# minhtrangvy/distributed_bitcoin_minter

Measured on AMD Instinct MI355X. Metric: GH/s (SHA-256 "msg nonce" min-search) at 1/2/4/8 MI355X; % of int32 VALU peak, higher is better.
Workload: dtype u32

## Files before the change

### distributed_bitcoin_minter_amd/csrc/bm_kernels.hpp

```cpp
#pragma once
#include <hip/hip_runtime.h>

#include <cstdint>
#include <type_traits>

#include "bm_common.h"
#include "bm_sha256.hpp"

namespace bm {

#define BM_DEV __device__ __forceinline__

template <int B, int E, class F>
BM_DEV void static_for(F&& f) {
    if constexpr (B < E) {
        f(std::integral_constant<int, B>{});
        static_for<B + 1, E>(f);
    }
}

BM_DEV uint32_t rotr(uint32_t x, uint32_t n) { return __builtin_amdgcn_alignbit(x, x, n); }

BM_DEV uint32_t xor3(uint32_t a, uint32_t b, uint32_t c) {
    if (__builtin_constant_p(a) && __builtin_constant_p(b) && __builtin_constant_p(c)) return a ^ b ^ c;
    return __builtin_amdgcn_bitop3_b32(a, b, c, 0x96);
}
BM_DEV uint32_t ch(uint32_t e, uint32_t f, uint32_t g) {
    if (__builtin_constant_p(e) && __builtin_constant_p(f) && __builtin_constant_p(g)) return (e & f) ^ (~e & g);
    return __builtin_amdgcn_bitop3_b32(e, f, g, 0xCA);
}
BM_DEV uint32_t maj(uint32_t a, uint32_t b, uint32_t c) {
    if (__builtin_constant_p(a) && __builtin_constant_p(b) && __builtin_constant_p(c))
        return (a & b) ^ (a & c) ^ (b & c);
    return __builtin_amdgcn_bitop3_b32(a, b, c, 0xE8);
}
BM_DEV uint32_t bsig0(uint32_t a) { return xor3(rotr(a, 2), rotr(a, 13), rotr(a, 22)); }
BM_DEV uint32_t bsig1(uint32_t e) { return xor3(rotr(e, 6), rotr(e, 11), rotr(e, 25)); }
BM_DEV uint32_t ssig0(uint32_t x) { return xor3(rotr(x, 7), rotr(x, 18), x >> 3); }
BM_DEV uint32_t ssig1(uint32_t x) { return xor3(rotr(x, 17), rotr(x, 19), x >> 10); }

template <int T>
BM_DEV void sha_round(uint32_t (&s)[8], uint32_t w) {
    uint32_t& a = s[(0 - T) & 7];
    uint32_t& b = s[(1 - T) & 7];
    uint32_t& c = s[(2 - T) & 7];
    uint32_t& d = s[(3 - T) & 7];
    uint32_t& e = s[(4 - T) & 7];
    uint32_t& f = s[(5 - T) & 7];
    uint32_t& g = s[(6 - T) & 7];
    uint32_t& h = s[(7 - T) & 7];
    const uint32_t t1 = h + bsig1(e) + ch(e, f, g) + (kK256[T] + w);
    d += t1;
    h = t1 + bsig0(a) + maj(a, b, c);
}

#ifndef BM_PAD_ADD3S
#define BM_PAD_ADD3S 1
#endif

BM_DEV uint32_t add3_sgpr(uint32_t a, uint32_t s, uint32_t b) {
    uint32_t r;
    asm("v_add3_u32 %0, %1, %2, %3" : "=v"(r) : "v"(a), "s"(s), "v"(b));
    return r;
}

template <int T, bool KW_SGPR = false>
BM_DEV void sha_round_kw(uint32_t (&s)[8], uint32_t kw) {
    uint32_t& a = s[(0 - T) & 7];
    uint32_t& b = s[(1 - T) & 7];
    uint32_t& c = s[(2 - T) & 7];
    uint32_t& d = s[(3 - T) & 7];
    uint32_t& e = s[(4 - T) & 7];
    uint32_t& f = s[(5 - T) & 7];
    uint32_t& g = s[(6 - T) & 7];
    uint32_t& h = s[(7 - T) & 7];
    uint32_t t1;
    if constexpr (KW_SGPR && BM_PAD_ADD3S)
        t1 = add3_sgpr(h, kw, ch(e, f, g)) + bsig1(e);
    else
        t1 = h + bsig1(e) + ch(e, f, g) + kw;
    d += t1;
    h = t1 + bsig0(a) + maj(a, b, c);
}

template <int R0, int R1>
BM_DEV void sha_rounds(uint32_t (&s)[8], uint32_t (&w)[16]) {
    static_for<R0, R1>([&](auto I) {
        constexpr int t = decltype(I)::value;
        if constexpr (t >= 16)
            w[t & 15] = ssig1(w[(t - 2) & 15]) + w[(t - 7) & 15] + ssig0(w[(t - 15) & 15]) + w[t & 15];
        sha_round<t>(s, w[t & 15]);
    });
}

BM_DEV uint32_t ssig0_uniform(uint32_t x) {
    return ((x >> 7) | (x << 25)) ^ ((x >> 18) | (x << 14)) ^ (x >> 3);
}

#ifndef BM_PIN
#define BM_PIN 1
#endif

BM_DEV uint32_t ssig0_salu(uint32_t x) {
    uint32_t r, t0, t1, t2;
    asm("s_lshr_b32 %1, %4, 7\n\t"
        "s_lshl_b32 %2, %4, 25\n\t"
        "s_or_b32 %1, %1, %2\n\t"
        "s_lshr_b32 %2, %4, 18\n\t"
        "s_lshl_b32 %3, %4, 14\n\t"
        "s_or_b32 %2, %2, %3\n\t"
        "s_xor_b32 %1, %1, %2\n\t"
        "s_lshr_b32 %2, %4, 3\n\t"
        "s_xor_b32 %0, %1, %2"
        : "=s"(r), "=&s"(t0), "=&s"(t1), "=&s"(t2)
        : "s"(x)
        : "scc");
    return r;
}

BM_DEV uint32_t vgpr_copy(uint32_t x) {
    uint32_t r;
    asm("v_mov_b32 %0, %1" : "=v"(r) : "s"(x));
    return r;
}

template <int R0, int V>
BM_DEV uint32_t sha_rounds_h0(uint32_t (&s)[8], uint32_t (&w)[16], uint32_t s0v, uint32_t h0_add) {
    static_assert(R0 <= V && V >= 1 && V <= 15, "varying word");
    static_for<R0, 63>([&](auto I) {
        constexpr int t = decltype(I)::value;
        if constexpr (t >= 16) {
            uint32_t s0;
            if constexpr (t - 15 == V)
                s0 = s0v;
            else
                s0 = ssig0(w[(t - 15) & 15]);
            w[t & 15] = ssig1(w[(t - 2) & 15]) + w[(t - 7) & 15] + s0 + w[t & 15];
        }
        sha_round<t>(s, w[t & 15]);
    });
    w[15] = ssig1(w[13]) + w[8] + ssig0(w[0]) + w[15];
    const uint32_t a = s[1], b = s[2], c = s[3], e = s[5], f = s[6], g = s[7], h = s[0];
    const uint32_t t1 = h + bsig1(e) + ch(e, f, g) + (kK256[63] + h0_add) + w[15];
    return t1 + bsig0(a) + maj(a, b, c);
}

BM_DEV void sha_compress(uint32_t (&st)[8], uint32_t (&w)[16]) {
    uint32_t s[8];
#pragma unroll
    for (int i = 0; i < 8; ++i) s[i] = st[i];
    sha_rounds<0, 64>(s, w);
#pragma unroll
    for (int i = 0; i < 8; ++i) st[i] += s[i];
}

template <int P, bool PADB>
constexpr int64_t tail_word(int k) {
    constexpr int LW = P / 4;
    if (k == LW + 1 && (P % 4) == 3 && P != 63) return 0x80000000ll;
    if (!PADB && k == 15) return -1;
    return 0;
}

template <int P, int NBV>
BM_DEV void add_task_digits(uint32_t (&W)[16 * NBV], uint64_t t, uint32_t ms, uint32_t nd) {
    uint64_t x = t;
    static_for<1, 20>([&](auto I) {
        constexpr int i = decltype(I)::value;
        constexpr int pos = 64 * (NBV - 1) + P - i;
        if constexpr (pos >= 0) {
            if (i >= (int)ms && i < (int)nd) {
                const uint64_t q = x / 10u;
                const uint32_t d = (uint32_t)(x - q * 10u);
                x = q;
                W[pos >> 2] += d << (8 * (3 - (pos & 3)));
            }
        }
    });
}

BM_DEV bool lex_less(uint64_t h1, uint64_t n1, uint64_t h2, uint64_t n2) {
    return h1 < h2 || (h1 == h2 && n1 < n2);
}

template <int XOR>
BM_DEV uint64_t swizzle_xor_u64(uint64_t v) {
    constexpr int pat = (XOR << 10) | 0x1F;
    const uint32_t lo = (uint32_t)__builtin_amdgcn_ds_swizzle((int)(uint32_t)v, pat);
    const uint32_t hi = (uint32_t)__builtin_amdgcn_ds_swizzle((int)(uint32_t)(v >> 32), pat);
    return ((uint64_t)hi << 32) | lo;
}

BM_DEV uint64_t readlane_u64(uint64_t v, int lane) {
    const uint32_t lo = (uint32_t)__builtin_amdgcn_readlane((int)(uint32_t)v, lane);
    const uint32_t hi = (uint32_t)__builtin_amdgcn_readlane((int)(uint32_t)(v >> 32), lane);
    return ((uint64_t)hi << 32) | lo;
}

BM_DEV void wave_min(uint64_t& h, uint64_t& n) {
    static_for<0, 5>([&](auto I) {
        constexpr int x = 1 << decltype(I)::value;
        const uint64_t oh = swizzle_xor_u64<x>(h), on = swizzle_xor_u64<x>(n);
        if (lex_less(oh, on, h, n)) {
            h = oh;
            n = on;
        }
    });
    const uint64_t h0 = readlane_u64(h, 0), n0 = readlane_u64(n, 0);
    const uint64_t h1 = readlane_u64(h, 32), n1 = readlane_u64(n, 32);
    if (lex_less(h1, n1, h0, n0)) {
        h = h1;
        n = n1;
    } else {
        h = h0;
        n = n0;
    }
}

template <int NT>
BM_DEV bool block_min(uint64_t& h, uint64_t& n) {
    constexpr int NWAVE = NT / 64;
    __shared__ Partial sh[NWAVE];
    wave_min(h, n);
    const int wave = threadIdx.x >> 6;
    if ((threadIdx.x & 63) == 0) sh[wave] = Partial{h, n};
    __syncthreads();
    if (threadIdx.x == 0) {
#pragma unroll
        for (int i = 1; i < NWAVE; ++i)
            if (lex_less(sh[i].hash, sh[i].nonce, h, n)) {
                h = sh[i].hash;
                n = sh[i].nonce;
            }
        return true;
    }
    return false;
}

BM_DEV uint64_t readfirstlane_u64(uint64_t v) {
    const uint32_t lo = (uint32_t)__builtin_amdgcn_readfirstlane((int)(uint32_t)v);
    const uint32_t hi = (uint32_t)__builtin_amdgcn_readfirstlane((int)(uint32_t)(v >> 32));
    return ((uint64_t)hi << 32) | lo;
}

#ifndef BM_FOLD
#define BM_FOLD 1
#endif
#ifndef BM_WAVES_MAIN
#define BM_WAVES_MAIN 7
#endif
#ifndef BM_WAVES_PAD
#define BM_WAVES_PAD 5
#endif
#ifndef BM_WAVES_NBV2
#define BM_WAVES_NBV2 7
#endif
#ifndef BM_NBV2_TIGHT
#define BM_NBV2_TIGHT 1
#endif
constexpr bool nbv2_tight(int P) { return BM_NBV2_TIGHT && P == 4; }
constexpr int search_waves(int P, int NBV) {
    return (NBV == 1 && P >= 55) ? BM_WAVES_PAD
                                 : (NBV == 2 ? (nbv2_tight(P) ? 6 : BM_WAVES_NBV2) : BM_WAVES_MAIN);
}
#ifndef BM_LDS_BEST
#define BM_LDS_BEST 0
#endif
#ifndef BM_CLOCK_PROBE
#define BM_CLOCK_PROBE 0
#endif
constexpr int kClockSlot = 16;
#ifndef BM_KATTR
#define BM_KATTR __attribute__((amdgpu_waves_per_eu(search_waves(P, NBV), 8)))
#endif

template <int P, int NBV, int PADK, bool TGT = false, bool HITS = false>
BM_DEV void search_body(const SearchArgs& A, Partial* __restrict__ part, unsigned long long* __restrict__ counter,
                        uint64_t target = 0, unsigned long long* hit = nullptr, Partial* hit_buf = nullptr,
                        uint64_t hit_cap = 0) {
    static_assert(!(TGT || HITS) || PADK == -1, "target and hits modes run the generic kernels");
    static_assert(!(TGT && HITS), "one mode");
    static_assert(P >= 0 && P < 64 && (NBV == 1 || (NBV == 2 && P <= 18)), "layout");
    constexpr int LW = P / 4;
    constexpr int BOFF = 16 * (NBV - 1);
    constexpr bool PADB = (NBV == 1) && (P >= 55);
    constexpr bool PADC = PADK >= 0;
    static_assert(!PADC || (PADB && PADK <= kMaxPadPrefixBlocks), "PADK is a padding-block layout");
    constexpr bool TWOW = (P % 4 == 0) && (LW >= 1);
    constexpr bool kFold = BM_FOLD && !PADB && LW >= 1 && !(NBV == 1 && (P == 53 || P == 54)) &&
                           !(NBV == 2 && P >= 17);
    constexpr bool kPin = BM_PIN && kFold && !(NBV == 1 && P >= 48);

    constexpr uint32_t inc0 = 1u << (8 * (3 - P % 4));
    constexpr uint32_t inc1 = (P % 4) >= 1 ? 1u << (8 * (4 - P % 4)) : 0u;
    constexpr uint32_t inc2 = (P % 4) >= 2 ? 1u << (8 * (5 - P % 4)) : 0u;
    constexpr uint32_t inc3 = (P % 4) >= 3 ? 1u << (8 * (6 - P % 4)) : 0u;

    uint64_t best_h = ~0ull, best_n = ~0ull;
    uint32_t bh = 0xFFFFFFFFu;
    const uint32_t thi = (uint32_t)(target >> 32);
    (void)thi;
#if BM_LDS_BEST
    __shared__ uint64_t lbest_h[kBlock], lbest_n[kBlock];
    lbest_h[threadIdx.x] = ~0ull;
    lbest_n[threadIdx.x] = ~0ull;
#endif

    const uint32_t S = A.S;
    const uint32_t n_in = TWOW ? 10u : S;
    const uint32_t n_out = TWOW ? S / 10u : 1u;
    const uint32_t lane = threadIdx.x & 63;
    const uint64_t ntask = A.t_end - A.t0;
    const uint64_t chunk = 64ull * A.chunk_m;

    if (BM_CLOCK_PROBE && blockIdx.x == 0 && threadIdx.x == 0) {
        counter[kClockSlot + 0] = __builtin_amdgcn_s_memtime();
        counter[kClockSlot + 1] = __builtin_amdgcn_s_memrealtime();
    }
    for (;;) {
        uint64_t base = 0;
        if constexpr (TGT) {
            uint64_t seen = 0;
            if (lane == 0) {
                base = atomicAdd(counter, (unsigned long long)chunk);
                seen = __hip_atomic_load(hit, __ATOMIC_RELAXED, __HIP_MEMORY_SCOPE_AGENT);
            }
            base = readfirstlane_u64(base);
            if (base >= ntask) break;
            seen = readfirstlane_u64(seen);
            if (seen < A.nonce_base || seen - A.nonce_base < (A.t0 + base) * (uint64_t)S) break;
        } else {
            if (lane == 0) base = atomicAdd(counter, (unsigned long long)chunk);
            base = readfirstlane_u64(base);
            if (base >= ntask) break;
        }
        for (uint32_t i = 0; i < A.chunk_m; ++i) {
            const uint64_t tt = base + 64ull * i + lane;
            if (tt >= ntask) break;
            const uint64_t t = A.t0 + tt;

            uint32_t W[16 * NBV];
            static_for<0, 16 * NBV>([&](auto K) { W[decltype(K)::value] = A.tmpl[decltype(K)::value]; });
            add_task_digits<P, NBV>(W, t, A.ms, A.nd);

            uint32_t st[8];
#pragma unroll
            for (int q = 0; q < 8; ++q) st[q] = PADK == 0 ? kIV256[q] : A.mid[q];
            if constexpr (NBV == 2) {
                uint32_t wa[16];
#pragma unroll
                for (int k = 0; k < 16; ++k) wa[k] = W[k];
                sha_compress(st, wa);
            }

            uint32_t wb[16];
            static_for<0, 16>([&](auto K) {
                constexpr int k = decltype(K)::value;
                if constexpr (k <= LW) {
                    wb[k] = W[BOFF + k];
                } else {
                    constexpr int64_t c = tail_word<P, PADB>(k);
                    if constexpr (c < 0)
                        wb[k] = (kPin && NBV == 1) ? vgpr_copy(A.tmpl[BOFF + k]) : A.tmpl[BOFF + k];
                    else
                        wb[k] = (uint32_t)c;
                }
            });
            constexpr int R0 = TWOW ? LW - 1 : LW;
            uint32_t s00[8];
#pragma unroll
            for (int q = 0; q < 8; ++q) s00[q] = st[q];
            sha_rounds<0, R0>(s00, wb);

            const uint64_t vbase = t * (uint64_t)S;
            for (uint32_t jo = 0; jo < n_out; ++jo) {
                uint32_t wo[16];
#pragma unroll
                for (int k = 0; k < 16; ++k) wo[k] = wb[k];
                uint32_t s0[8];
#pragma unroll
                for (int q = 0; q < 8; ++q) s0[q] = s00[q];
                if constexpr (TWOW) {
                    wo[LW - 1] = wb[LW - 1] + jo;
                    sha_rounds<LW - 1, LW>(s0, wo);
                }
                const uint32_t wl = wo[LW];
                const uint32_t s0wl = ssig0(wl);
                const uint32_t h0_add = (kPin && NBV == 1) ? vgpr_copy(st[0]) : st[0];
                const uint32_t h1_add = (kPin && NBV == 1) ? vgpr_copy(st[1]) : st[1];

                uint32_t J = 0, c0 = 0, c1 = 0, c2 = 0;
                for (uint32_t j = 0; j < n_in; ++j) {
                    uint32_t w[16];
#pragma unroll
                    for (int k = 0; k < 16; ++k) w[k] = wo[k];
                    w[LW] = wl + J;
                    uint32_t x[8];
#pragma unroll
                    for (int q = 0; q < 8; ++q) x[q] = s0[q];

                    uint32_t h0, h1;
                    if constexpr (kFold) {
                        const uint32_t s0J = kPin ? ssig0_salu(J) : ssig0_uniform(J);
                        h0 = sha_rounds_h0<LW, LW>(x, w, s0wl ^ s0J, h0_add);
                        h1 = h1_add + x[1];
                    } else if constexpr (PADB) {
                        sha_rounds<LW, 64>(x, w);
                        uint32_t y[8];
#pragma unroll
                        for (int q = 0; q < 8; ++q) y[q] = st[q] + x[q];
                        uint32_t z[8];
#pragma unroll
                        for (int q = 0; q < 8; ++q) z[q] = y[q];
                        static_for<0, 64>([&](auto I) {
                            constexpr int tt2 = decltype(I)::value;
                            if constexpr (PADC) {
                                constexpr uint32_t kw = kPadKW<P, (PADK > 0 ? PADK : 0)>.v[tt2];
                                sha_round_kw<tt2>(z, kw);
                            } else {
                                sha_round_kw<tt2, true>(z, A.padkw[tt2]);
                            }
                        });
                        h0 = y[0] + z[0];
                        h1 = y[1] + z[1];
                    } else {
                        sha_rounds<LW, 64>(x, w);
                        h0 = st[0] + x[0];
                        h1 = st[1] + x[1];
                    }

                    if (__builtin_expect(h0 <= bh, 0)) {
                        const uint64_t h = ((uint64_t)h0 << 32) | h1;
                        const uint64_t v = vbase + (uint64_t)jo * n_in + j;
                        if constexpr (TGT) {
                            if (h <= target && v >= A.vlo && v <= A.vhi)
                                atomicMin(hit, (unsigned long long)(A.nonce_base + v));
                        }
                        if constexpr (HITS) {
                            if (h <= target && v >= A.vlo && v <= A.vhi) {
                                const unsigned long long idx = atomicAdd(hit, 1ull);
                                if (idx < hit_cap) {
                                    using u64x2 = unsigned long long __attribute__((ext_vector_type(2)));
                                    *reinterpret_cast<u64x2*>(hit_buf + idx) = u64x2{h, A.nonce_base + v};
                                }
                            }
                        }
#if BM_LDS_BEST
                        if (h < lbest_h[threadIdx.x] && v >= A.vlo && v <= A.vhi) {
                            lbest_h[threadIdx.x] = h;
                            lbest_n[threadIdx.x] = A.nonce_base + v;
                            bh = HITS ? (h0 > thi ? h0 : thi) : h0;
                        }
#else
                        if (h < best_h && v >= A.vlo && v <= A.vhi) {
                            best_h = h;
                            best_n = A.nonce_base + v;
                            bh = HITS ? (h0 > thi ? h0 : thi) : h0;
                        }
#endif
                    }

                    J += inc0;
                    if (++c0 == 10u) {
                        c0 = 0;
                        J += inc1 - 10u * inc0;
                        if (++c1 == 10u) {
                            c1 = 0;
                            J += inc2 - 10u * inc1;
                            if (++c2 == 10u) {
                                c2 = 0;
                                J += inc3 - 10u * inc2;
                            }
                        }
                    }
                }
            }
        }
    }

    if (BM_CLOCK_PROBE && blockIdx.x == 0 && threadIdx.x == 0) {
        counter[kClockSlot + 2] = __builtin_amdgcn_s_memtime();
        counter[kClockSlot + 3] = __builtin_amdgcn_s_memrealtime();
    }
#if BM_LDS_BEST
    best_h = lbest_h[threadIdx.x];
    best_n = lbest_n[threadIdx.x];
#endif
    if (block_min<kBlock>(best_h, best_n)) part[A.part_off + blockIdx.x] = Partial{best_h, best_n};
}

template <int P, int NBV>
__global__ __launch_bounds__(kBlock) BM_KATTR void search_kernel(
    const SearchArgs A, Partial* __restrict__ part, unsigned long long* __restrict__ counter) {
    search_body<P, NBV, -1>(A, part, counter);
}

template <int P, int NBV = 1>
__global__ __launch_bounds__(kBlock) BM_KATTR void search_kernel_padc(
    const SearchArgs A, Partial* __restrict__ part, unsigned long long* __restrict__ counter) {
    static_assert(NBV == 1 && P >= 55, "padding-block layouts only");
    search_body<P, 1, 0>(A, part, counter);
}

template <int P, int K, int NBV = 1>
__global__ __launch_bounds__(kBlock) BM_KATTR void search_kernel_padk(
    const SearchArgs A, Partial* __restrict__ part, unsigned long long* __restrict__ counter) {
    static_assert(NBV == 1 && P >= 55 && K >= 1 && K <= kMaxPadPrefixBlocks, "padding-block layouts only");
    search_body<P, 1, K>(A, part, counter);
}

template <int P, int NBV>
__global__ __launch_bounds__(kBlock) BM_KATTR void target_kernel(
    const SearchArgs A, Partial* __restrict__ part, unsigned long long* __restrict__ counter, const uint64_t target,
    unsigned long long* __restrict__ hit) {
    search_body<P, NBV, -1, true>(A, part, counter, target, hit);
}

template <int P, int NBV>
__global__ __launch_bounds__(kBlock) BM_KATTR void hits_kernel(
    const SearchArgs A, Partial* __restrict__ part, unsigned long long* __restrict__ counter, const uint64_t target,
    unsigned long long* __restrict__ hit_count, Partial* __restrict__ hit_buf, const uint64_t hit_cap) {
    search_body<P, NBV, -1, false, true>(A, part, counter, target, hit_count, hit_buf, hit_cap);
}

}
```

Before: 52.28.

## Compute task digits once per wave and share best-hash threshold across lanes

```diff
diff --git a/distributed_bitcoin_minter_amd/csrc/bm_digits.hpp b/distributed_bitcoin_minter_amd/csrc/bm_digits.hpp
--- /dev/null
+++ b/distributed_bitcoin_minter_amd/csrc/bm_digits.hpp
@@ -0,0 +1,115 @@
+#pragma once
+#include <cstdint>
+
+#if defined(__HIPCC__) || defined(__CUDACC__)
+#define BM_DIGITS_FN __host__ __device__ __forceinline__
+#else
+#define BM_DIGITS_FN inline
+#endif
+#if defined(__clang__)
+#define BM_UNROLL _Pragma("unroll")
+#else
+#define BM_UNROLL
+#endif
+
+namespace bm {
+
+constexpr int kDigitWords = 5;
+
+constexpr int task_digit_words(int P, int NBV) {
+    const int E = 64 * (NBV - 1) + P;
+    return ((E < 19 ? E : 19) + 3) / 4;
+}
+
+BM_DIGITS_FN void pack9(uint32_t x, uint64_t& lo8, uint32_t& d8) {
+    uint64_t p = 0;
+    BM_UNROLL
+    for (int k = 0; k < 8; ++k) {
+        const uint32_t q = x / 10u;
+        p |= (uint64_t)(x - q * 10u) << (8 * k);
+        x = q;
+    }
+    lo8 = p;
+    d8 = x;
+}
+
+template <int NW>
+BM_DIGITS_FN void task_digits_uniform(uint64_t u, uint32_t (&T)[kDigitWords]) {
+    BM_UNROLL
+    for (int k = 0; k < kDigitWords; ++k) T[k] = 0;
+    if (NW == 0) return;
+    uint32_t l0, l1 = 0, l2 = 0;
+    if (NW < 3 || u < 1000000000ull) {
+        l0 = (uint32_t)u;
+    } else {
+        const uint64_t q = u / 1000000000ull;
+        l0 = (uint32_t)(u - q * 1000000000ull);
+        if (q < 1000000000ull) {
+            l1 = (uint32_t)q;
+        } else {
+            l2 = (uint32_t)(q / 1000000000ull);
+            l1 = (uint32_t)(q - (uint64_t)l2 * 1000000000ull);
+        }
+    }
+    uint64_t p0;
+    uint32_t e0;
+    pack9(l0, p0, e0);
+    T[0] = (uint32_t)p0;
+    T[1] = (uint32_t)(p0 >> 32);
+    T[2] = e0;
+    if (NW >= 3 && (l1 | l2) != 0) {
+        uint64_t p1;
+        uint32_t e1;
+        pack9(l1, p1, e1);
+        const uint32_t q2 = l2 / 10u;
+        T[2] |= (uint32_t)p1 << 8;
+        T[3] = (uint32_t)(p1 >> 24);
+        T[4] = (uint32_t)(p1 >> 56) | (e1 << 8) | ((l2 - q2 * 10u) << 16) | (q2 << 24);
+    }
+}
+
+BM_DIGITS_FN uint32_t lane_digits(uint32_t lane) {
+    const uint32_t q = lane / 10u;
+    return (lane - q * 10u) | (q << 8);
+}
+
+template <int NW>
+BM_DIGITS_FN void task_digits_add_lane(const uint32_t (&T)[kDigitWords], uint32_t lane2, uint32_t (&R)[kDigitWords]) {
+    uint32_t carry = 0;
+    BM_UNROLL
+    for (int k = 0; k < kDigitWords; ++k) {
+        if (k >= NW) {
+            R[k] = 0;
+            continue;
+        }
+        const uint64_t s = (uint64_t)T[k] + (k == 0 ? lane2 : 0u) + 0xF6F6F6F6u + carry;
+        carry = (uint32_t)(s >> 32);
+        const uint32_t x = (uint32_t)s;
+        const uint32_t h = x & 0x80808080u;
+        R[k] = x - (((h - (h >> 7)) | h) & 0xF6F6F6F6u);
+    }
+}
+
+template <int P, int NBV>
+BM_DIGITS_FN void place_task_digits(uint32_t (&W)[16 * NBV], const uint32_t (&R)[kDigitWords], uint32_t ms) {
+    constexpr int E = 64 * (NBV - 1) + P;
+    constexpr int NW = task_digit_words(P, NBV);
+    constexpr int c = 8 * (3 - E % 4);
+    if (NW == 0) return;
+    uint32_t Q[kDigitWords + 1];
+    const uint32_t sh = 32u - 8u * ms;
+    BM_UNROLL
+    for (int k = 0; k <= NW; ++k) {
+        const uint32_t hi = k < NW ? R[k] : 0u, lo = k > 0 ? R[k - 1] : 0u;
+        Q[k] = (uint32_t)((((uint64_t)hi << 32) | lo) >> sh);
+    }
+    BM_UNROLL
+    for (int k = 0; k <= NW + 1; ++k) {
+        const int idx = E / 4 - k;
+        if (idx < 0 || (c == 0 && k > NW)) break;
+        const uint32_t hi = k <= NW ? Q[k] : 0u, lo = k > 0 ? Q[k - 1] : 0u;
+        W[idx] += c == 0 ? hi : (hi << c) | (lo >> ((32 - c) & 31));
+    }
+}
+
+}
diff --git a/distributed_bitcoin_minter_amd/csrc/bm_kernels.hpp b/distributed_bitcoin_minter_amd/csrc/bm_kernels.hpp
--- a/distributed_bitcoin_minter_amd/csrc/bm_kernels.hpp
+++ b/distributed_bitcoin_minter_amd/csrc/bm_kernels.hpp
@@ -5,6 +5,7 @@
 #include <type_traits>
 
 #include "bm_common.h"
+#include "bm_digits.hpp"
 #include "bm_sha256.hpp"
 
 namespace bm {
@@ -163,7 +164,16 @@
 }
 
 template <int P, int NBV>
-BM_DEV void add_task_digits(uint32_t (&W)[16 * NBV], uint64_t t, uint32_t ms, uint32_t nd) {
+BM_DEV void add_task_digits(uint32_t (&W)[16 * NBV], uint64_t u, uint32_t lane2, uint32_t ms) {
+    constexpr int NW = task_digit_words(P, NBV);
+    uint32_t T[kDigitWords], R[kDigitWords];
+    task_digits_uniform<NW>(u, T);
+    task_digits_add_lane<NW>(T, lane2, R);
+    place_task_digits<P, NBV>(W, R, ms);
+}
+
+template <int P, int NBV>
+BM_DEV void add_task_digits_div(uint32_t (&W)[16 * NBV], uint64_t t, uint32_t ms, uint32_t nd) {
     uint64_t x = t;
     static_for<1, 20>([&](auto I) {
         constexpr int i = decltype(I)::value;
@@ -263,6 +273,12 @@
     return (NBV == 1 && P >= 55) ? BM_WAVES_PAD
                                  : (NBV == 2 ? (nbv2_tight(P) ? 6 : BM_WAVES_NBV2) : BM_WAVES_MAIN);
 }
+#ifndef BM_TASK_DIGITS_SALU
+#define BM_TASK_DIGITS_SALU 1
+#endif
+#ifndef BM_WAVE_BH
+#define BM_WAVE_BH 1
+#endif
 #ifndef BM_LDS_BEST
 #define BM_LDS_BEST 0
 #endif
@@ -290,6 +306,8 @@
     constexpr bool kFold = BM_FOLD && !PADB && LW >= 1 && !(NBV == 1 && (P == 53 || P == 54)) &&
                            !(NBV == 2 && P >= 17);
     constexpr bool kPin = BM_PIN && kFold && !(NBV == 1 && P >= 48);
+    constexpr bool kSaluDigits = BM_TASK_DIGITS_SALU && !PADB;
+    constexpr bool kWaveBh = BM_WAVE_BH && !PADB;
 
     constexpr uint32_t inc0 = 1u << (8 * (3 - P % 4));
     constexpr uint32_t inc1 = (P % 4) >= 1 ? 1u << (8 * (4 - P % 4)) : 0u;
@@ -310,6 +328,7 @@
     const uint32_t n_in = TWOW ? 10u : S;
     const uint32_t n_out = TWOW ? S / 10u : 1u;
     const uint32_t lane = threadIdx.x & 63;
+    const uint32_t lane2 = lane_digits(lane);
     const uint64_t ntask = A.t_end - A.t0;
     const uint64_t chunk = 64ull * A.chunk_m;
 
@@ -341,7 +360,10 @@
 
             uint32_t W[16 * NBV];
             static_for<0, 16 * NBV>([&](auto K) { W[decltype(K)::value] = A.tmpl[decltype(K)::value]; });
-            add_task_digits<P, NBV>(W, t, A.ms, A.nd);
+            if constexpr (kSaluDigits)
+                add_task_digits<P, NBV>(W, A.t0 + base + 64ull * i, lane2, A.ms);
+            else
+                add_task_digits_div<P, NBV>(W, t, A.ms, A.nd);
 
             uint32_t st[8];
 #pragma unroll
@@ -429,35 +451,77 @@
                         h1 = st[1] + x[1];
                     }
 
-                    if (__builtin_expect(h0 <= bh, 0)) {
-                        const uint64_t h = ((uint64_t)h0 << 32) | h1;
-                        const uint64_t v = vbase + (uint64_t)jo * n_in + j;
-                        if constexpr (TGT) {
-                            if (h <= target && v >= A.vlo && v <= A.vhi)
-                                atomicMin(hit, (unsigned long long)(A.nonce_base + v));
+                    if constexpr (!kWaveBh) {
+                        if (__builtin_expect(h0 <= bh, 0)) {
+                            const uint64_t h = ((uint64_t)h0 << 32) | h1;
+                            const uint64_t v = vbase + (uint64_t)jo * n_in + j;
+                            if constexpr (TGT) {
+                                if (h <= target && v >= A.vlo && v <= A.vhi)
+                                    atomicMin(hit, (unsigned long long)(A.nonce_base + v));
+                            }
+                            if constexpr (HITS) {
+                                if (h <= target && v >= A.vlo && v <= A.vhi) {
+                                    const unsigned long long idx = atomicAdd(hit, 1ull);
+                                    if (idx < hit_cap) {
+                                        using u64x2 = unsigned long long __attribute__((ext_vector_type(2)));
+                                        *reinterpret_cast<u64x2*>(hit_buf + idx) = u64x2{h, A.nonce_base + v};
+                                    }
+                                }
+                            }
+#if BM_LDS_BEST
+                            if (h < lbest_h[threadIdx.x] && v >= A.vlo && v <= A.vhi) {
+                                lbest_h[threadIdx.x] = h;
+                                lbest_n[threadIdx.x] = A.nonce_base + v;
+                                bh = HITS ? (h0 > thi ? h0 : thi) : h0;
+                            }
+#else
+                            if (h < best_h && v >= A.vlo && v <= A.vhi) {
+                                best_h = h;
+                                best_n = A.nonce_base + v;
+                                bh = HITS ? (h0 > thi ? h0 : thi) : h0;
+                            }
+#endif
                         }
-                        if constexpr (HITS) {
-                            if (h <= target && v >= A.vlo && v <= A.vhi) {
-                                const unsigned long long idx = atomicAdd(hit, 1ull);
-                                if (idx < hit_cap) {
-                                    using u64x2 = unsigned long long __attribute__((ext_vector_type(2)));
-                                    *reinterpret_cast<u64x2*>(hit_buf + idx) = u64x2{h, A.nonce_base + v};
+                    } else
+                    if (__builtin_expect(__builtin_amdgcn_ballot_w64(h0 <= bh) != 0, 0)) {
+                        uint32_t acc = 0xFFFFFFFFu;
+                        if (h0 <= bh) {
+                            const uint64_t h = ((uint64_t)h0 << 32) | h1;
+                            const uint64_t v = vbase + (uint64_t)jo * n_in + j;
+                            if constexpr (TGT) {
+                                if (h <= target && v >= A.vlo && v <= A.vhi)
+                                    atomicMin(hit, (unsigned long long)(A.nonce_base + v));
+                            }
+                            if constexpr (HITS) {
+                                if (h <= target && v >= A.vlo && v <= A.vhi) {
+                                    const unsigned long long idx = atomicAdd(hit, 1ull);
+                                    if (idx < hit_cap) {
+                                        using u64x2 = unsigned long long __attribute__((ext_vector_type(2)));
+                                        *reinterpret_cast<u64x2*>(hit_buf + idx) = u64x2{h, A.nonce_base + v};
+                                    }
                                 }
                             }
+#if BM_LDS_BEST
+                            if (h < lbest_h[threadIdx.x] && v >= A.vlo && v <= A.vhi) {
+                                lbest_h[threadIdx.x] = h;
+                                lbest_n[threadIdx.x] = A.nonce_base + v;
+                                acc = h0;
+                            }
+#else
+                            if (h < best_h && v >= A.vlo && v <= A.vhi) {
+                                best_h = h;
+                                best_n = A.nonce_base + v;
+                                acc = h0;
+                            }
+#endif
                         }
-#if BM_LDS_BEST
-                        if (h < lbest_h[threadIdx.x] && v >= A.vlo && v <= A.vhi) {
-                            lbest_h[threadIdx.x] = h;
-                            lbest_n[threadIdx.x] = A.nonce_base + v;
-                            bh = HITS ? (h0 > thi ? h0 : thi) : h0;
+                        const uint64_t am = __builtin_amdgcn_ballot_w64(acc != 0xFFFFFFFFu);
+                        if (am != 0) {
+                            const uint32_t wa = (uint32_t)__builtin_amdgcn_readlane((int)acc, __builtin_ctzll(am));
+                            uint32_t nb = acc < wa ? acc : wa;
+                            if ((TGT || HITS) && nb < thi) nb = thi;
+                            bh = nb < bh ? nb : bh;
                         }
-#else
-                        if (h < best_h && v >= A.vlo && v <= A.vhi) {
-                            best_h = h;
-                            best_n = A.nonce_base + v;
-                            bh = HITS ? (h0 > thi ? h0 : thi) : h0;
-                        }
-#endif
                     }
 
                     J += inc0;
```

New measurement: 52.24. Within noise of the previous version (-0.1%).
